# tencent-ailab/pika

Hardware: NVIDIA H100
Metric: utterances/sec RNN-T train step (T=1000,U=150,V=6k) (higher is better)
Workload: dtype bf16

## Files before the change

pika_b200/csrc/common.cuh:

```cuda
#pragma once
#include <cuda.h>
#include <cuda_bf16.h>
#include <cuda_runtime.h>
#include <stdint.h>

#define PK_DEVICE __device__ __forceinline__

namespace pk {

void set_last_error(const char* fmt, ...);
#define PK_CHECK_ARG(cond, msg)                                       \
    do {                                                              \
        if (!(cond)) {                                                \
            pk::set_last_error("%s:%d: %s", __FILE__, __LINE__, msg); \
            return -1;                                                \
        }                                                             \
    } while (0)
#define PK_CHECK_CUDA(expr)                                                                     \
    do {                                                                                        \
        cudaError_t e__ = (expr);                                                               \
        if (e__ != cudaSuccess) {                                                               \
            pk::set_last_error("%s:%d: CUDA error %s", __FILE__, __LINE__, cudaGetErrorString(e__)); \
            return -2;                                                                          \
        }                                                                                       \
// ... 52 lines not shown
    x ^= x >> 15; x *= 0x85EBCA77u; x ^= x >> 13;
    return ((x & 0xFFFFu) >= thresh16 ? 1u : 0u) | ((x >> 16) >= thresh16 ? 2u : 0u);
}
__host__ __device__ inline uint32_t drop_thresh16_of(float p) {
    if (p <= 0.f) return 0u;
    const double t = (double)p * 65536.0 + 0.5;
    const uint32_t r = t >= 65535.0 ? 65535u : (uint32_t)t;
    return r == 0 ? 1u : r;
}
__host__ __device__ inline float drop_scale16_of(uint32_t thresh16) { return thresh16 ? 1.f / (1.f - (float)thresh16 / 65536.f) : 1.f; }

PK_DEVICE float warp_sum(float v) {
#pragma unroll
    for (int o = 16; o > 0; o >>= 1) v += __shfl_xor_sync(0xffffffffu, v, o);
    return v;
}
PK_DEVICE float warp_max(float v) {
#pragma unroll
    for (int o = 16; o > 0; o >>= 1) v = fmaxf(v, __shfl_xor_sync(0xffffffffu, v, o));
    return v;
}

PK_DEVICE uint32_t smem_u32(const void* p) { return (uint32_t)__cvta_generic_to_shared(p); }

PK_DEVICE bool elect_one() {
    uint32_t pred;
    asm volatile(
        "{\n\t.reg .pred p;\n\t.reg .b32 r;\n\t"
        "elect.sync r|p, 0xffffffff;\n\t"
        "selp.u32 %0, 1, 0, p;\n\t}\n"
        : "=r"(pred));
    return pred != 0;
}

PK_DEVICE void mbar_init(uint64_t* bar, uint32_t count) {
    asm volatile("mbarrier.init.shared::cta.b64 [%0], %1;" ::"r"(smem_u32(bar)), "r"(count));
}
PK_DEVICE void mbar_fence_init() { asm volatile("fence.mbarrier_init.release.cluster;" ::: "memory"); }
PK_DEVICE void mbar_arrive_expect_tx(uint64_t* bar, uint32_t bytes) {
    asm volatile("mbarrier.arrive.expect_tx.shared::cta.b64 _, [%0], %1;" ::"r"(smem_u32(bar)), "r"(bytes)
                 : "memory");
}
PK_DEVICE void mbar_arrive(uint64_t* bar) {
    asm volatile("mbarrier.arrive.shared::cta.b64 _, [%0];" ::"r"(smem_u32(bar)) : "memory");
}
PK_DEVICE bool mbar_try_wait(uint64_t* bar, uint32_t parity) {
    uint32_t done;
    asm volatile(
        "{\n\t.reg .pred p;\n\t"
        "mbarrier.try_wait.parity.shared::cta.b64 p, [%1], %2;\n\t"
        "selp.u32 %0, 1, 0, p;\n\t}\n"
        : "=r"(done)
        : "r"(smem_u32(bar)), "r"(parity)
        : "memory");
    return done != 0;
}
PK_DEVICE void mbar_wait(uint64_t* bar, uint32_t parity) {
    while (!mbar_try_wait(bar, parity)) {
    }
}

PK_DEVICE void tma_prefetch_desc(const CUtensorMap* m) {
    asm volatile("prefetch.tensormap [%0];" ::"l"(reinterpret_cast<uint64_t>(m)) : "memory");
}
PK_DEVICE void tma_load_4d(void* smem_dst, const CUtensorMap* m, uint64_t* bar, int c0, int c1, int c2, int c3) {
    asm volatile(
        "cp.async.bulk.tensor.4d.shared::cluster.global.tile.mbarrier::complete_tx::bytes"
        " [%0], [%1, {%3, %4, %5, %6}], [%2];" ::"r"(smem_u32(smem_dst)),
        "l"(reinterpret_cast<uint64_t>(m)), "r"(smem_u32(bar)), "r"(c0), "r"(c1), "r"(c2), "r"(c3)
        : "memory");
}
PK_DEVICE void tma_load_3d(void* smem_dst, const CUtensorMap* m, uint64_t* bar, int c0, int c1, int c2) {
    asm volatile(
        "cp.async.bulk.tensor.3d.shared::cluster.global.tile.mbarrier::complete_tx::bytes"
        " [%0], [%1, {%3, %4, %5}], [%2];" ::"r"(smem_u32(smem_dst)),
        "l"(reinterpret_cast<uint64_t>(m)), "r"(smem_u32(bar)), "r"(c0), "r"(c1), "r"(c2)
        : "memory");
}
PK_DEVICE void bulk_load(void* smem_dst, const void* gsrc, uint32_t bytes, uint64_t* bar) {
    asm volatile("cp.async.bulk.shared::cluster.global.mbarrier::complete_tx::bytes [%0], [%1], %2, [%3];" ::"r"(smem_u32(smem_dst)),
                 "l"(reinterpret_cast<uint64_t>(gsrc)), "r"(bytes), "r"(smem_u32(bar))
                 : "memory");
}
PK_DEVICE void tma_store_4d(const CUtensorMap* m, const void* smem_src, int c0, int c1, int c2, int c3) {
    asm volatile(
        "cp.async.bulk.tensor.4d.global.shared::cta.tile.bulk_group [%0, {%2, %3, %4, %5}], [%1];" ::"l"(
            reinterpret_cast<uint64_t>(m)),
        "r"(smem_u32(smem_src)), "r"(c0), "r"(c1), "r"(c2), "r"(c3)
        : "memory");
}
PK_DEVICE void tma_reduce_add_4d(const CUtensorMap* m, const void* smem_src, int c0, int c1, int c2, int c3) {
    asm volatile(
        "cp.reduce.async.bulk.tensor.4d.global.shared::cta.add.tile.bulk_group [%0, {%2, %3, %4, %5}], [%1];" ::"l"(
            reinterpret_cast<uint64_t>(m)),
        "r"(smem_u32(smem_src)), "r"(c0), "r"(c1), "r"(c2), "r"(c3)
        : "memory");
}
constexpr uint64_t kL2EvictNormal = 0x1000000000000000ull;
constexpr uint64_t kL2EvictFirst = 0x12F0000000000000ull;
constexpr uint64_t kL2EvictLast = 0x14F0000000000000ull;
PK_DEVICE void tma_load_4d_hint(void* smem_dst, const CUtensorMap* m, uint64_t* bar, int c0, int c1, int c2, int c3, uint64_t pol) {
    asm volatile(
        "cp.async.bulk.tensor.4d.shared::cluster.global.tile.mbarrier::complete_tx::bytes.L2::cache_hint"
        " [%0], [%1, {%3, %4, %5, %6}], [%2], %7;" ::"r"(smem_u32(smem_dst)),
        "l"(reinterpret_cast<uint64_t>(m)), "r"(smem_u32(bar)), "r"(c0), "r"(c1), "r"(c2), "r"(c3), "l"(pol)
        : "memory");
}
PK_DEVICE void tma_store_4d_hint(const CUtensorMap* m, const void* smem_src, int c0, int c1, int c2, int c3, uint64_t pol) {
    asm volatile(
        "cp.async.bulk.tensor.4d.global.shared::cta.tile.bulk_group.L2::cache_hint [%0, {%2, %3, %4, %5}], [%1], %6;" ::"l"(
            reinterpret_cast<uint64_t>(m)),
        "r"(smem_u32(smem_src)), "r"(c0), "r"(c1), "r"(c2), "r"(c3), "l"(pol)
        : "memory");
}
PK_DEVICE void tma_store_commit() { asm volatile("cp.async.bulk.commit_group;" ::: "memory"); }
template <int N> PK_DEVICE void tma_store_wait_read() {
    asm volatile("cp.async.bulk.wait_group.read %0;" ::"n"(N) : "memory");
}
template <int N> PK_DEVICE void tma_store_wait() { asm volatile("cp.async.bulk.wait_group %0;" ::"n"(N) : "memory"); }
PK_DEVICE void fence_proxy_async_smem() { asm volatile("fence.proxy.async.shared::cta;" ::: "memory"); }

PK_DEVICE uint64_t make_smem_desc_sw128(uint32_t smem_addr, uint32_t lbo_bytes, uint32_t sbo_bytes) {
    uint64_t d = 0;
    d |= (uint64_t)((smem_addr >> 4) & 0x3FFF);
    d |= (uint64_t)((lbo_bytes >> 4) & 0x3FFF) << 16;
    d |= (uint64_t)((sbo_bytes >> 4) & 0x3FFF) << 32;
    d |= (uint64_t)1 << 62;
    return d;
}
PK_DEVICE void wgmma_fence() { asm volatile("wgmma.fence.sync.aligned;" ::: "memory"); }
PK_DEVICE void wgmma_commit() { asm volatile("wgmma.commit_group.sync.aligned;" ::: "memory"); }
template <int N> PK_DEVICE void wgmma_wait() { asm volatile("wgmma.wait_group.sync.aligned %0;" ::"n"(N) : "memory"); }
template <int R> PK_DEVICE void wgmma_fence_acc(float (&d)[R]) {
#pragma unroll
    for (int i = 0; i < R; ++i) asm volatile("" : "+f"(d[i])::"memory");
}
template <int N> PK_DEVICE void setmaxnreg_inc() { asm volatile("setmaxnreg.inc.sync.aligned.u32 %0;" ::"n"(N)); }
template <int N> PK_DEVICE void setmaxnreg_dec() { asm volatile("setmaxnreg.dec.sync.aligned.u32 %0;" ::"n"(N)); }

template <int TA, int TB> PK_DEVICE void wgmma_ss_n64(float (&d)[32], uint64_t a, uint64_t b, uint32_t acc) {
    asm volatile(
        "{\n\t.reg .pred p;\n\tsetp.ne.b32 p, %34, 0;\n\t"
        "wgmma.mma_async.sync.aligned.m64n64k16.f32.bf16.bf16 {%0, %1, %2, %3, %4, %5, %6, %7, %8, %9, %10, %11, %12, %13, %14, %15, %16, %17, %18, %19, %20, %21, %22, %23, %24, %25, %26, %27, %28, %29, %30, %31}, %32, %33, p, 1, 1, %35, %36;\n\t}\n"
        : "+f"(d[0]), "+f"(d[1]), "+f"(d[2]), "+f"(d[3]), "+f"(d[4]), "+f"(d[5]), "+f"(d[6]), "+f"(d[7]), "+f"(d[8]), "+f"(d[9]), "+f"(d[10]), "+f"(d[11]), "+f"(d[12]), "+f"(d[13]), "+f"(d[14]), "+f"(d[15]), "+f"(d[16]), "+f"(d[17]), "+f"(d[18]), "+f"(d[19]), "+f"(d[20]), "+f"(d[21]), "+f"(d[22]), "+f"(d[23]), "+f"(d[24]), "+f"(d[25]), "+f"(d[26]), "+f"(d[27]), "+f"(d[28]), "+f"(d[29]), "+f"(d[30]), "+f"(d[31])
        : "l"(a), "l"(b), "r"(acc), "n"(TA), "n"(TB));
}
template <int TB> PK_DEVICE void wgmma_rs_n64(float (&d)[32], const uint32_t (&a)[4], uint64_t b, uint32_t acc) {
    asm volatile(
        "{\n\t.reg .pred p;\n\tsetp.ne.b32 p, %37, 0;\n\t"
        "wgmma.mma_async.sync.aligned.m64n64k16.f32.bf16.bf16 {%0, %1, %2, %3, %4, %5, %6, %7, %8, %9, %10, %11, %12, %13, %14, %15, %16, %17, %18, %19, %20, %21, %22, %23, %24, %25, %26, %27, %28, %29, %30, %31}, {%32, %33, %34, %35}, %36, p, 1, 1, %38;\n\t}\n"
        : "+f"(d[0]), "+f"(d[1]), "+f"(d[2]), "+f"(d[3]), "+f"(d[4]), "+f"(d[5]), "+f"(d[6]), "+f"(d[7]), "+f"(d[8]), "+f"(d[9]), "+f"(d[10]), "+f"(d[11]), "+f"(d[12]), "+f"(d[13]), "+f"(d[14]), "+f"(d[15]), "+f"(d[16]), "+f"(d[17]), "+f"(d[18]), "+f"(d[19]), "+f"(d[20]), "+f"(d[21]), "+f"(d[22]), "+f"(d[23]), "+f"(d[24]), "+f"(d[25]), "+f"(d[26]), "+f"(d[27]), "+f"(d[28]), "+f"(d[29]), "+f"(d[30]), "+f"(d[31])
        : "r"(a[0]), "r"(a[1]), "r"(a[2]), "r"(a[3]), "l"(b), "r"(acc), "n"(TB));
}
template <int TA, int TB> PK_DEVICE void wgmma_ss_n128(float (&d)[64], uint64_t a, uint64_t b, uint32_t acc) {
    asm volatile(
        "{\n\t.reg .pred p;\n\tsetp.ne.b32 p, %66, 0;\n\t"
        "wgmma.mma_async.sync.aligned.m64n128k16.f32.bf16.bf16 {%0, %1, %2, %3, %4, %5, %6, %7, %8, %9, %10, %11, %12, %13, %14, %15, %16, %17, %18, %19, %20, %21, %22, %23, %24, %25, %26, %27, %28, %29, %30, %31, %32, %33, %34, %35, %36, %37, %38, %39, %40, %41, %42, %43, %44, %45, %46, %47, %48, %49, %50, %51, %52, %53, %54, %55, %56, %57, %58, %59, %60, %61, %62, %63}, %64, %65, p, 1, 1, %67, %68;\n\t}\n"
        : "+f"(d[0]), "+f"(d[1]), "+f"(d[2]), "+f"(d[3]), "+f"(d[4]), "+f"(d[5]), "+f"(d[6]), "+f"(d[7]), "+f"(d[8]), "+f"(d[9]), "+f"(d[10]), "+f"(d[11]), "+f"(d[12]), "+f"(d[13]), "+f"(d[14]), "+f"(d[15]), "+f"(d[16]), "+f"(d[17]), "+f"(d[18]), "+f"(d[19]), "+f"(d[20]), "+f"(d[21]), "+f"(d[22]), "+f"(d[23]), "+f"(d[24]), "+f"(d[25]), "+f"(d[26]), "+f"(d[27]), "+f"(d[28]), "+f"(d[29]), "+f"(d[30]), "+f"(d[31]), "+f"(d[32]), "+f"(d[33]), "+f"(d[34]), "+f"(d[35]), "+f"(d[36]), "+f"(d[37]), "+f"(d[38]), "+f"(d[39]), "+f"(d[40]), "+f"(d[41]), "+f"(d[42]), "+f"(d[43]), "+f"(d[44]), "+f"(d[45]), "+f"(d[46]), "+f"(d[47]), "+f"(d[48]), "+f"(d[49]), "+f"(d[50]), "+f"(d[51]), "+f"(d[52]), "+f"(d[53]), "+f"(d[54]), "+f"(d[55]), "+f"(d[56]), "+f"(d[57]), "+f"(d[58]), "+f"(d[59]), "+f"(d[60]), "+f"(d[61]), "+f"(d[62]), "+f"(d[63])
        : "l"(a), "l"(b), "r"(acc), "n"(TA), "n"(TB));
}
template <int TA, int TB> PK_DEVICE void wgmma_ss_n256(float (&d)[128], uint64_t a, uint64_t b, uint32_t acc) {
    asm volatile(
        "{\n\t.reg .pred p;\n\tsetp.ne.b32 p, %130, 0;\n\t"
        "wgmma.mma_async.sync.aligned.m64n256k16.f32.bf16.bf16 {%0, %1, %2, %3, %4, %5, %6, %7, %8, %9, %10, %11, %12, %13, %14, %15, %16, %17, %18, %19, %20, %21, %22, %23, %24, %25, %26, %27, %28, %29, %30, %31, %32, %33, %34, %35, %36, %37, %38, %39, %40, %41, %42, %43, %44, %45, %46, %47, %48, %49, %50, %51, %52, %53, %54, %55, %56, %57, %58, %59, %60, %61, %62, %63, %64, %65, %66, %67, %68, %69, %70, %71, %72, %73, %74, %75, %76, %77, %78, %79, %80, %81, %82, %83, %84, %85, %86, %87, %88, %89, %90, %91, %92, %93, %94, %95, %96, %97, %98, %99, %100, %101, %102, %103, %104, %105, %106, %107, %108, %109, %110, %111, %112, %113, %114, %115, %116, %117, %118, %119, %120, %121, %122, %123, %124, %125, %126, %127}, %128, %129, p, 1, 1, %131, %132;\n\t}\n"
        : "+f"(d[0]), "+f"(d[1]), "+f"(d[2]), "+f"(d[3]), "+f"(d[4]), "+f"(d[5]), "+f"(d[6]), "+f"(d[7]), "+f"(d[8]), "+f"(d[9]), "+f"(d[10]), "+f"(d[11]), "+f"(d[12]), "+f"(d[13]), "+f"(d[14]), "+f"(d[15]), "+f"(d[16]), "+f"(d[17]), "+f"(d[18]), "+f"(d[19]), "+f"(d[20]), "+f"(d[21]), "+f"(d[22]), "+f"(d[23]), "+f"(d[24]), "+f"(d[25]), "+f"(d[26]), "+f"(d[27]), "+f"(d[28]), "+f"(d[29]), "+f"(d[30]), "+f"(d[31]), "+f"(d[32]), "+f"(d[33]), "+f"(d[34]), "+f"(d[35]), "+f"(d[36]), "+f"(d[37]), "+f"(d[38]), "+f"(d[39]), "+f"(d[40]), "+f"(d[41]), "+f"(d[42]), "+f"(d[43]), "+f"(d[44]), "+f"(d[45]), "+f"(d[46]), "+f"(d[47]), "+f"(d[48]), "+f"(d[49]), "+f"(d[50]), "+f"(d[51]), "+f"(d[52]), "+f"(d[53]), "+f"(d[54]), "+f"(d[55]), "+f"(d[56]), "+f"(d[57]), "+f"(d[58]), "+f"(d[59]), "+f"(d[60]), "+f"(d[61]), "+f"(d[62]), "+f"(d[63]), "+f"(d[64]), "+f"(d[65]), "+f"(d[66]), "+f"(d[67]), "+f"(d[68]), "+f"(d[69]), "+f"(d[70]), "+f"(d[71]), "+f"(d[72]), "+f"(d[73]), "+f"(d[74]), "+f"(d[75]), "+f"(d[76]), "+f"(d[77]), "+f"(d[78]), "+f"(d[79]), "+f"(d[80]), "+f"(d[81]), "+f"(d[82]), "+f"(d[83]), "+f"(d[84]), "+f"(d[85]), "+f"(d[86]), "+f"(d[87]), "+f"(d[88]), "+f"(d[89]), "+f"(d[90]), "+f"(d[91]), "+f"(d[92]), "+f"(d[93]), "+f"(d[94]), "+f"(d[95]), "+f"(d[96]), "+f"(d[97]), "+f"(d[98]), "+f"(d[99]), "+f"(d[100]), "+f"(d[101]), "+f"(d[102]), "+f"(d[103]), "+f"(d[104]), "+f"(d[105]), "+f"(d[106]), "+f"(d[107]), "+f"(d[108]), "+f"(d[109]), "+f"(d[110]), "+f"(d[111]), "+f"(d[112]), "+f"(d[113]), "+f"(d[114]), "+f"(d[115]), "+f"(d[116]), "+f"(d[117]), "+f"(d[118]), "+f"(d[119]), "+f"(d[120]), "+f"(d[121]), "+f"(d[122]), "+f"(d[123]), "+f"(d[124]), "+f"(d[125]), "+f"(d[126]), "+f"(d[127])
        : "l"(a), "l"(b), "r"(acc), "n"(TA), "n"(TB));
// ... 99 lines not shown
```

pika_b200/csrc/rnnt_loss.cu:

```cuda
#include <algorithm>
#include <cstdlib>

#include "../../include/pika_b200.h"
#include "common.cuh"

namespace pk {
void count_launch();

constexpr float kLog2e = 1.4426950408889634f;
constexpr float kLn2 = 0.6931471805599453f;

template <typename T> struct Vec16;
template <> struct Vec16<__nv_bfloat16> {
    static constexpr int N = 8;
    PK_DEVICE static void unpack(const uint4& q, float (&f)[8]) {
        f[0] = bf16lo(q.x); f[1] = bf16hi(q.x); f[2] = bf16lo(q.y); f[3] = bf16hi(q.y);
        f[4] = bf16lo(q.z); f[5] = bf16hi(q.z); f[6] = bf16lo(q.w); f[7] = bf16hi(q.w);
    }
    PK_DEVICE static uint4 pack(const float (&f)[8]) {
        return make_uint4(pack_bf16x2(f[0], f[1]), pack_bf16x2(f[2], f[3]), pack_bf16x2(f[4], f[5]), pack_bf16x2(f[6], f[7]));
    }
    PK_DEVICE static float vmax(const uint4& q) {
        const __nv_bfloat162 a = __hmax2(*reinterpret_cast<const __nv_bfloat162*>(&q.x), *reinterpret_cast<const __nv_bfloat162*>(&q.y));
        const __nv_bfloat162 b = __hmax2(*reinterpret_cast<const __nv_bfloat162*>(&q.z), *reinterpret_cast<const __nv_bfloat162*>(&q.w));
// ... 295 lines not shown
    for (int o = 1; o < 32; o <<= 1) {
        const int y = __shfl_up_sync(0xffffffffu, x, o);
        if (lane >= o) x += y;
    }
    if (lane == 31) s_warp[w] = x;
    __syncthreads();
    if (w == 0) {
        int s = s_warp[lane];
#pragma unroll
        for (int o = 1; o < 32; o <<= 1) {
            const int y = __shfl_up_sync(0xffffffffu, s, o);
            if (lane >= o) s += y;
        }
        s_warp[lane] = s;
    }
    __syncthreads();
    const int r = x - v + (w > 0 ? s_warp[w - 1] : 0);
    *total = s_warp[31];
    __syncthreads();
    return r;
}

PK_DEVICE int tile_kept(const float* gb, const float* gl, long long rows, long long r0, bool (&keep)[SCAN_PER_THREAD]) {
    int n = 0;
#pragma unroll
    for (int k = 0; k < SCAN_PER_THREAD; ++k) {
        const long long r = r0 + (long long)threadIdx.x * SCAN_PER_THREAD + k;
        keep[k] = r < rows && grad_row_kept(gb[r], gl[r]);
        n += keep[k];
    }
    return n;
}

__global__ void __launch_bounds__(SCAN_THREADS) grad_rows_count_kernel(const float* __restrict__ gb, const float* __restrict__ gl,
                                                                       long long rows, int* __restrict__ tile_count) {
    __shared__ int s_warp[32];
    bool keep[SCAN_PER_THREAD];
    int total;
    block_exclusive_scan(tile_kept(gb, gl, rows, (long long)blockIdx.x * SCAN_TILE, keep), s_warp, &total);
    if (threadIdx.x == 0) tile_count[blockIdx.x] = total;
}

template <typename T>
__global__ void __launch_bounds__(SCAN_THREADS) grad_rows_scan_kernel(int* __restrict__ tile_count, int n_tiles, int* __restrict__ count,
                                                                      long long rows, T* dz_c, int ldv, T* h_c, int H) {
    __shared__ int s_warp[32];
    __shared__ int s_carry;
    if (threadIdx.x == 0) s_carry = 0;
    __syncthreads();
    for (int i0 = 0; i0 < n_tiles; i0 += SCAN_THREADS) {
        const int i = i0 + threadIdx.x;
        const int v = i < n_tiles ? tile_count[i] : 0;
        int total;
        const int ex = block_exclusive_scan(v, s_warp, &total);
        if (i < n_tiles) tile_count[i] = s_carry + ex;
        __syncthreads();
        if (threadIdx.x == 0) s_carry += total;
        __syncthreads();
    }
    const long long kept = s_carry;
    if (threadIdx.x == 0) *count = (int)kept;
    const long long tail = min(rows, (kept + 63) / 64 * 64);
    for (long long r = kept; r < tail; ++r) {
        for (int c = threadIdx.x; c < ldv; c += SCAN_THREADS) dz_c[r * ldv + c] = from_f32<T>(0.f);
        for (int c = threadIdx.x; c < H; c += SCAN_THREADS) h_c[r * H + c] = from_f32<T>(0.f);
    }
}

__global__ void __launch_bounds__(SCAN_THREADS) grad_rows_map_kernel(const float* __restrict__ gb, const float* __restrict__ gl,
                                                                     long long rows, const int* __restrict__ tile_off, int* __restrict__ map) {
    __shared__ int s_warp[32];
    bool keep[SCAN_PER_THREAD];
    const long long r0 = (long long)blockIdx.x * SCAN_TILE;
    int total;
    int idx = tile_off[blockIdx.x] + block_exclusive_scan(tile_kept(gb, gl, rows, r0, keep), s_warp, &total);
#pragma unroll
    for (int k = 0; k < SCAN_PER_THREAD; ++k) {
        const long long r = r0 + (long long)threadIdx.x * SCAN_PER_THREAD + k;
        if (r < rows) map[r] = keep[k] ? idx++ : -1;
    }
}

constexpr int GRAD_THREADS = 256;
template <typename T> struct GradCfg { static constexpr int MAXG = 32 / Vec16<T>::N; };
template <typename T, int GRAD_RU, int MINB, bool COMPACT, bool ROWY = false>
__global__ void __launch_bounds__(GRAD_THREADS, MINB) rnnt_grad_kernel(const T* logits, const int* __restrict__ labels,
                                                                    const int* __restrict__ label_lens, RnntDims d,
                                                                    const float* __restrict__ lse_in, const float* __restrict__ gb_in,
                                                                    const float* __restrict__ gl_in, T* dlogits, float* __restrict__ colsum,
                                                                    long long rows_per_cta, const int* __restrict__ row_map,
                                                                    const T* __restrict__ h, T* __restrict__ h_c, int H,
                                                                    const int* __restrict__ row_y = nullptr) {
    constexpr int VN = Vec16<T>::N;
    constexpr int GRAD_MAXG = GradCfg<T>::MAXG;
    extern __shared__ float gsm[];
    float* s_gb = gsm;
    float* s_gl = gsm + rows_per_cta;
    float* s_l2 = gsm + 2 * rows_per_cta;
    int* s_y = reinterpret_cast<int*>(gsm + 3 * rows_per_cta);
    int* s_map = reinterpret_cast<int*>(gsm + 4 * rows_per_cta);
    const long long rows = (long long)d.B * d.T * d.U1;
    const long long r0 = (long long)blockIdx.x * rows_per_cta;
    const long long r1 = min(rows, r0 + rows_per_cta);
    const int nvec_ld = d.ldv / VN;
    const int tid = threadIdx.x;
    for (long long row = r0 + tid; row < r1; row += GRAD_THREADS) {
        const int i = (int)(row - r0);
        s_gb[i] = gb_in[row];
        s_gl[i] = gl_in[row];
        s_l2[i] = lse_in[row] * kLog2e;
        if (ROWY) {
            s_y[i] = row_y[row];
        } else {
            const int u = (int)(row % d.U1);
            const int b = (int)(row / ((long long)d.T * d.U1));
            s_y[i] = (u < label_lens[b]) ? labels[(size_t)b * d.ld_labels + u] : -1;
        }
        if (COMPACT) s_map[i] = row_map[row];
    }
    __syncthreads();
    const int h_vec = COMPACT ? H / 8 : 0;
    float cs[GRAD_MAXG][VN];
#pragma unroll
    for (int gq = 0; gq < GRAD_MAXG; ++gq)
#pragma unroll
        for (int e = 0; e < VN; ++e) cs[gq][e] = 0.f;
    for (long long rb = r0; rb < r1; rb += GRAD_RU) {
        uint4 q[GRAD_RU][GRAD_MAXG];
        uint4 hq[GRAD_RU];
#pragma unroll
        for (int k = 0; k < GRAD_RU; ++k) {
            const long long row = rb + k;
            if (row < r1 && (COMPACT ? s_map[row - r0] >= 0 : (s_gb[row - r0] != 0.f || s_gl[row - r0] != 0.f))) {
                const uint4* vp = reinterpret_cast<const uint4*>(logits + row * (long long)d.ldv);
#pragma unroll
                for (int gq = 0; gq < GRAD_MAXG; ++gq) {
                    const int i = tid + gq * GRAD_THREADS;
                    if (i < nvec_ld) q[k][gq] = ld_plain(vp + i);
                }
                if (COMPACT && tid < h_vec) hq[k] = ld_stream(reinterpret_cast<const uint4*>(h + row * (long long)H) + tid);
            }
        }
#pragma unroll
        for (int k = 0; k < GRAD_RU; ++k) {
            const long long row = rb + k;
            if (row >= r1) continue;
            const float gb = s_gb[row - r0], gl = s_gl[row - r0];
            long long orow = row;
            if (COMPACT) {
                orow = s_map[row - r0];
                if (orow < 0) continue;
                if (tid < h_vec) st_stream(reinterpret_cast<uint4*>(h_c + orow * H) + tid, hq[k]);
            }
            uint4* op = reinterpret_cast<uint4*>(dlogits + orow * (long long)d.ldv);
            if (gb == 0.f && gl == 0.f) {
#pragma unroll
                for (int gq = 0; gq < GRAD_MAXG; ++gq) {
                    const int i = tid + gq * GRAD_THREADS;
                    if (i < nvec_ld) st_stream(op + i, make_uint4(0, 0, 0, 0));
                }
                continue;
            }
            const int y = s_y[row - r0];
            const float l2 = s_l2[row - r0];
            const float gsum = -(gb + gl);
#pragma unroll
            for (int gq = 0; gq < GRAD_MAXG; ++gq) {
                const int i = tid + gq * GRAD_THREADS;
                if (i < nvec_ld) {
                    float f[VN];
                    Vec16<T>::unpack(q[k][gq], f);
#pragma unroll
                    for (int e = 0; e < VN; ++e) f[e] = ex2_approx(fmaf(f[e], kLog2e, -l2)) * gsum;
                    const int v0 = i * VN;
                    if (v0 == 0) f[0] += gb;
                    if (y >= v0 && y < v0 + VN) {
#pragma unroll
                        for (int e = 0; e < VN; ++e) if (v0 + e == y) f[e] += gl;
                    }
                    if (v0 + VN > d.V) {
#pragma unroll
                        for (int e = 0; e < VN; ++e) if (v0 + e >= d.V) f[e] = 0.f;
                    }
                    const uint4 packed = Vec16<T>::pack(f);
                    st_stream(op + i, packed);
                    if (colsum) {
                        float w[VN];
                        Vec16<T>::unpack(packed, w);
#pragma unroll
                        for (int e = 0; e < VN; ++e) cs[gq][e] += w[e];
                    }
                }
            }
        }
    }
    if (colsum) {
        float* part = colsum + (size_t)blockIdx.x * d.ldv;
#pragma unroll
        for (int gq = 0; gq < GRAD_MAXG; ++gq) {
            const int i = tid + gq * GRAD_THREADS;
            if (i < nvec_ld) {
#pragma unroll
                for (int e = 0; e < VN; ++e) part[i * VN + e] = cs[gq][e];
            }
        }
    }
}

__global__ void __launch_bounds__(256) colsum_partials_kernel(const float* __restrict__ part, int n_part, int ld, float* __restrict__ out) {
    __shared__ float sm[8][33];
    const int tx = threadIdx.x & 31, ty = threadIdx.x >> 5;
    const int c = blockIdx.x * 32 + tx;
    float a = 0.f;
    if (c < ld) {
        const int per = (n_part + 7) / 8;
        const int i0 = ty * per, i1 = min(n_part, i0 + per);
        float a0 = 0.f, a1 = 0.f, a2 = 0.f, a3 = 0.f;
        int i = i0;
        for (; i + 4 <= i1; i += 4) {
            a0 += part[(size_t)(i + 0) * ld + c]; a1 += part[(size_t)(i + 1) * ld + c];
            a2 += part[(size_t)(i + 2) * ld + c]; a3 += part[(size_t)(i + 3) * ld + c];
        }
        for (; i < i1; ++i) a0 += part[(size_t)i * ld + c];
        a = (a0 + a1) + (a2 + a3);
    }
    sm[ty][tx] = a;
    __syncthreads();
    if (ty == 0 && c < ld) {
        float t = sm[0][tx];
#pragma unroll
        for (int k = 1; k < 8; ++k) t += sm[k][tx];
        out[c] = t;
    }
}

template <typename T>
__global__ void __launch_bounds__(256) pruned_row_lse_kernel(const T* __restrict__ logits, const int* __restrict__ frame_lens,
                                                             const int* __restrict__ label_lens, const int* __restrict__ bounds, int Tt,
                                                             int R, int V, int ldv, long long rows, const float2* __restrict__ parts,
                                                             int n_parts, float* __restrict__ lse_out) {
    constexpr int VN = Vec16<T>::N;
    const int lane = threadIdx.x & 31;
    const long long n_warps = (long long)gridDim.x * (blockDim.x >> 5);
    for (long long row = (long long)blockIdx.x * (blockDim.x >> 5) + (threadIdx.x >> 5); row < rows; row += n_warps) {
        const long long bt = row / R;
        const int r = (int)(row - bt * R), t = (int)(bt % Tt), b = (int)(bt / Tt);
        if (t >= frame_lens[b] || bounds[bt] < 0 || bounds[bt] + r > label_lens[b]) continue;
        float lse;
        if (parts != nullptr) {
            float m = -INFINITY, sum = 0.f;
            for (int i = 0; i < n_parts; ++i) m = fmaxf(m, parts[(size_t)i * rows + row].x);
            for (int i = 0; i < n_parts; ++i) { const float2 ps = parts[(size_t)i * rows + row]; sum += ps.y * exp2f(ps.x - m); }
            lse = (m + log2f(sum)) * kLn2;
        } else {
            const T* rp = logits + row * (long long)ldv;
            float m = -INFINITY, sum = 0.f;
            const int nfull = V / VN;
            for (int i = lane; i < nfull; i += 32) {
                float f[VN];
                Vec16<T>::unpack(ld_plain(reinterpret_cast<const uint4*>(rp) + i), f);
#pragma unroll
                for (int e = 0; e < VN; ++e) {
                    const float x = f[e] * kLog2e;
                    if (x > m) { sum *= exp2f(m - x); m = x; }
                    sum += exp2f(x - m);
                }
            }
            for (int v = nfull * VN + lane; v < V; v += 32) {
                const float x = to_f32<T>(rp[v]) * kLog2e;
                if (x > m) { sum *= exp2f(m - x); m = x; }
                sum += exp2f(x - m);
            }
            const float mw = warp_max(m);
            sum = (m == -INFINITY) ? 0.f : sum * exp2f(m - mw);
            sum = warp_sum(sum);
            lse = (mw + log2f(sum)) * kLn2;
        }
        if (lane == 0) lse_out[row] = lse;
    }
}

template <typename T>
__global__ void __launch_bounds__(256) pruned_tables_kernel(const T* __restrict__ logits, const int* __restrict__ labels,
                                                            const int* __restrict__ frame_lens, const int* __restrict__ label_lens,
                                                            const int* __restrict__ bounds, RnntDims d, int R,
                                                            const float* __restrict__ lse, float* __restrict__ lpb_skew,
                                                            float* __restrict__ lpl_skew) {
    const long long n = (long long)d.B * d.T * d.U1;
    for (long long i = (long long)blockIdx.x * blockDim.x + threadIdx.x; i < n; i += (long long)gridDim.x * blockDim.x) {
// ... 71 lines not shown
    PK_CHECK_ARG(cpt <= LAT_MAX_CPT, "U too large for the lattice kernel (U+1 <= 2048)");
    static bool configured = false;
    if (!configured) {
        PK_CHECK_CUDA(cudaFuncSetAttribute(rnnt_lattice_kernel, cudaFuncAttributeMaxDynamicSharedMemorySize,
                                           2 * 2 * (LAT_MAX_G * LAT_MAX_CPT + 2) * (int)sizeof(lat_t)));
        configured = true;
    }
    rnnt_lattice_kernel<<<d.B, 2 * G, lat_smem, stream>>>(frame_lens, label_lens, d, G, cpt, lpb, lpl, alpha, beta, grad_scale,
                                                       costs, gb, gl);
    PK_CHECK_LAUNCH(); count_launch();
    return 0;
}

static int rnnt_loss_impl(const void* logits, int dtype, const int* labels, const int* frame_lens,
                          const int* label_lens, int B, int T, int U1, int V, int ldv, int ld_labels,
                          const float* grad_scale, float* costs, void* dlogits, float* dlogits_colsum, void* workspace,
                          long long workspace_bytes, const float* row_lse, int n_parts, int* row_map, int* row_count,
                          const void* h, int H, void* h_c, void* stream_v) {
    using namespace pk;
    cudaStream_t stream = reinterpret_cast<cudaStream_t>(stream_v);
    PK_CHECK_ARG(dtype == PK_F32 || dtype == PK_BF16, "bad dtype");
    PK_CHECK_ARG(B > 0 && T > 0 && U1 > 0 && V > 1, "bad dims");
    const int vn = dtype == PK_F32 ? 4 : 8;
    PK_CHECK_ARG(ldv >= V && ldv % vn == 0, "ldv must be >= V and a multiple of 16 bytes");
    PK_CHECK_ARG((reinterpret_cast<uintptr_t>(logits) & 15) == 0, "logits not 16B aligned");
    PK_CHECK_ARG(dlogits == nullptr || (reinterpret_cast<uintptr_t>(dlogits) & 15) == 0, "dlogits not 16B aligned");
    PK_CHECK_ARG(workspace_bytes >= pk_rnnt_loss_workspace_bytes(B, T, U1), "workspace too small");
    RnntDims d{B, T, U1, V, ldv, ld_labels, T + U1 - 1};
    const size_t skew = (size_t)B * d.ND * U1, nodes = (size_t)B * T * U1;
    double* wsd = reinterpret_cast<double*>(workspace);
    double* alpha = wsd; double* beta = alpha + skew;
    float* lpb = reinterpret_cast<float*>(beta + skew); float* lpl = lpb + skew;
    float* lse = lpl + skew; float* gb = lse + nodes; float* gl = gb + nodes;

    const long long rows = (long long)nodes;
    const int warps_per_cta = 8;
    long long want = (rows + warps_per_cta - 1) / warps_per_cta;
    const long long cap = (long long)num_sms() * 8 * 4;
    const int grid = (int)(want < cap ? want : cap);
    if (row_lse != nullptr) {
        PK_CHECK_ARG(n_parts >= 1, "n_parts must be >= 1");
        const int fgrid = (int)((rows + 255) / 256 < (long long)num_sms() * 8 ? (rows + 255) / 256 : (long long)num_sms() * 8);
        if (dtype == PK_BF16)
            rnnt_rowfinish_kernel<__nv_bfloat16><<<fgrid, 256, 0, stream>>>(reinterpret_cast<const __nv_bfloat16*>(logits), labels, frame_lens,
                                                                           label_lens, d, reinterpret_cast<const float2*>(row_lse), n_parts,
                                                                           lse, lpb, lpl);
        else
            rnnt_rowfinish_kernel<float><<<fgrid, 256, 0, stream>>>(reinterpret_cast<const float*>(logits), labels, frame_lens, label_lens, d,
                                                                   reinterpret_cast<const float2*>(row_lse), n_parts, lse, lpb, lpl);
    } else if (dtype == PK_BF16)
        rnnt_rowstats_kernel<__nv_bfloat16><<<grid, 256, 0, stream>>>(reinterpret_cast<const __nv_bfloat16*>(logits), labels,
                                                                     frame_lens, label_lens, d, lse, lpb, lpl);
    else
        rnnt_rowstats_kernel<float><<<grid, 256, 0, stream>>>(reinterpret_cast<const float*>(logits), labels, frame_lens,
                                                              label_lens, d, lse, lpb, lpl);
    PK_CHECK_LAUNCH(); count_launch();
    {
        const int rc = launch_lattice(frame_lens, label_lens, d, lpb, lpl, alpha, beta, grad_scale, costs, gb, gl, stream);
        if (rc) return rc;
    }
    if (dlogits != nullptr) {
        PK_CHECK_ARG(ldv <= 8192, "V too large for the gradient kernel (V <= 8192)");
        int ggrid; long long rpc;
        rnnt_grad_grid(rows, &rpc, &ggrid);
        float* cs_part = nullptr;
        if (dlogits_colsum) {
            const long long base_bytes = pk_rnnt_loss_workspace_bytes(B, T, U1);
            PK_CHECK_ARG(workspace_bytes >= base_bytes + (long long)ggrid * ldv * 4,
                         "workspace too small for the column sums (add pk_rnnt_loss_colsum_workspace_bytes)");
            cs_part = reinterpret_cast<float*>(reinterpret_cast<unsigned char*>(workspace) + base_bytes);
        }
        if (row_map != nullptr) {
            const int n_tiles = (int)((rows + SCAN_TILE - 1) / SCAN_TILE);
            int* tile_count = reinterpret_cast<int*>(alpha);
            grad_rows_count_kernel<<<n_tiles, SCAN_THREADS, 0, stream>>>(gb, gl, rows, tile_count);
            PK_CHECK_LAUNCH(); count_launch();
            grad_rows_scan_kernel<__nv_bfloat16><<<1, SCAN_THREADS, 0, stream>>>(tile_count, n_tiles, row_count, rows,
                                                                                 reinterpret_cast<__nv_bfloat16*>(dlogits), ldv,
                                                                                 reinterpret_cast<__nv_bfloat16*>(h_c), H);
            PK_CHECK_LAUNCH(); count_launch();
            grad_rows_map_kernel<<<n_tiles, SCAN_THREADS, 0, stream>>>(gb, gl, rows, tile_count, row_map);
            PK_CHECK_LAUNCH(); count_launch();
        }
        const size_t gsmem = (size_t)rpc * (row_map != nullptr ? 20 : 16);
#define PK_GRAD_LAUNCH(TT, RU, MB, CP)                                                                                     \
        rnnt_grad_kernel<TT, RU, MB, CP><<<ggrid, GRAD_THREADS, gsmem, stream>>>(reinterpret_cast<const TT*>(logits), labels, label_lens, d, \
                                                                                lse, gb, gl, reinterpret_cast<TT*>(dlogits), cs_part, rpc,  \
                                                                                row_map, reinterpret_cast<const TT*>(h),                    \
                                                                                reinterpret_cast<TT*>(h_c), H)
        if (row_map != nullptr) PK_GRAD_LAUNCH(__nv_bfloat16, 2, 3, true);
        else if (dtype == PK_BF16) PK_GRAD_LAUNCH(__nv_bfloat16, 2, 3, false);
        else PK_GRAD_LAUNCH(float, 2, 2, false);
#undef PK_GRAD_LAUNCH
        PK_CHECK_LAUNCH(); count_launch();
        if (dlogits_colsum) {
            colsum_partials_kernel<<<(ldv + 31) / 32, 256, 0, stream>>>(cs_part, ggrid, ldv, dlogits_colsum);
            PK_CHECK_LAUNCH(); count_launch();
        }
    }
    return 0;
}

extern "C" int pk_rnnt_loss_fwd_bwd(const void* logits, int dtype, const int* labels, const int* frame_lens,
                                    const int* label_lens, int B, int T, int U1, int V, int ldv, int ld_labels,
                                    const float* grad_scale, float* costs, void* dlogits, float* dlogits_colsum, void* workspace,
                                    long long workspace_bytes, void* stream) {
    return rnnt_loss_impl(logits, dtype, labels, frame_lens, label_lens, B, T, U1, V, ldv, ld_labels, grad_scale, costs, dlogits,
                          dlogits_colsum, workspace, workspace_bytes, nullptr, 0, nullptr, nullptr, nullptr, 0, nullptr, stream);
}

extern "C" int pk_rnnt_loss_fwd_bwd_lse(const void* logits, int dtype, const int* labels, const int* frame_lens,
                                        const int* label_lens, int B, int T, int U1, int V, int ldv, int ld_labels,
                                        const float* grad_scale, float* costs, void* dlogits, float* dlogits_colsum, void* workspace,
                                        long long workspace_bytes, const float* row_lse, int n_parts, void* stream) {
    PK_CHECK_ARG(row_lse != nullptr, "row_lse is null");
    return rnnt_loss_impl(logits, dtype, labels, frame_lens, label_lens, B, T, U1, V, ldv, ld_labels, grad_scale, costs, dlogits,
                          dlogits_colsum, workspace, workspace_bytes, row_lse, n_parts, nullptr, nullptr, nullptr, 0, nullptr, stream);
}

extern "C" int pk_rnnt_loss_fwd_bwd_compact(const void* logits, int dtype, const int* labels, const int* frame_lens,
                                            const int* label_lens, int B, int T, int U1, int V, int ldv, int ld_labels,
                                            const float* grad_scale, float* costs, void* dz_c, float* dlogits_colsum, void* workspace,
                                            long long workspace_bytes, const float* row_lse, int n_parts, const void* h, int H,
                                            void* h_c, int* row_map, int* row_count, void* stream) {
    PK_CHECK_ARG(dtype == PK_BF16, "the compacted gradient is bf16 only");
    PK_CHECK_ARG(dz_c != nullptr && row_map != nullptr && row_count != nullptr && h != nullptr && h_c != nullptr, "null pointer");
    PK_CHECK_ARG(H > 0 && H % 8 == 0 && H / 8 <= pk::GRAD_THREADS, "H must be a multiple of 8, <= 2048");
    PK_CHECK_ARG(dz_c != logits, "dz_c must not alias the logits");
    PK_CHECK_ARG((reinterpret_cast<uintptr_t>(h) & 15) == 0 && (reinterpret_cast<uintptr_t>(h_c) & 15) == 0, "h / h_c not 16B aligned");
    return rnnt_loss_impl(logits, dtype, labels, frame_lens, label_lens, B, T, U1, V, ldv, ld_labels, grad_scale, costs, dz_c,
                          dlogits_colsum, workspace, workspace_bytes, row_lse, n_parts, row_map, row_count, h, H, h_c, stream);
}

static long long lattice_ws_bytes(int B, int T, int U1) { return 2 * (long long)B * ((long long)T + U1 - 1) * U1 * 8; }
extern "C" int pk_rnnt_lattice_workspace(int B, int T, int U1, long long* bytes) {
    PK_CHECK_ARG(B > 0 && T > 0 && U1 > 0 && bytes != nullptr, "bad dims or null pointer");
    *bytes = lattice_ws_bytes(B, T, U1);
    return 0;
}

extern "C" int pk_rnnt_lattice(const int* frame_lens, const int* label_lens, int B, int T, int U1, const float* lpb_skew,
                               const float* lpl_skew, const float* grad_scale, float* costs, float* gb, float* gl, void* workspace,
                               long long workspace_bytes, void* stream) {
    using namespace pk;
    PK_CHECK_ARG(B > 0 && T > 0 && U1 > 0, "bad dims");
    PK_CHECK_ARG(lpb_skew && lpl_skew && costs && gb && gl && workspace, "null pointer");
    PK_CHECK_ARG(workspace_bytes >= lattice_ws_bytes(B, T, U1), "workspace too small");
    RnntDims d{B, T, U1, 2, 2, 1, T + U1 - 1};
    const size_t skew = (size_t)B * d.ND * U1;
    double* alpha = reinterpret_cast<double*>(workspace);
    return launch_lattice(frame_lens, label_lens, d, lpb_skew, lpl_skew, alpha, alpha + skew, grad_scale, costs, gb, gl,
                          reinterpret_cast<cudaStream_t>(stream));
}

static long long pruned_ws_parts(int B, int T, int U1, int R, int ldv, long long* colsum_off) {
    const long long skew = (long long)B * ((long long)T + U1 - 1) * U1, nodes = (long long)B * T * U1, rows = (long long)B * T * R;
    const long long base = 2 * skew * 8 + 2 * skew * 4 + 2 * nodes * 4 + 4 * rows * 4;
    const long long off = (base + 255) / 256 * 256;
    int ggrid; long long rpc;
    rnnt_grad_grid(rows, &rpc, &ggrid);
    if (colsum_off) *colsum_off = off;
    return off + (long long)ggrid * ldv * 4;
}
extern "C" int pk_rnnt_pruned_loss_workspace(int B, int T, int U1, int R, int ldv, long long* bytes) {
    PK_CHECK_ARG(B > 0 && T > 0 && U1 > 0 && R >= 1 && ldv > 0 && bytes != nullptr, "bad dims or null pointer");
    *bytes = pruned_ws_parts(B, T, U1, R, ldv, nullptr);
    return 0;
}

extern "C" int pk_rnnt_pruned_loss(const void* logits, int dtype, const int* labels, const int* frame_lens, const int* label_lens,
                                   const int* bounds, int B, int T, int U1, int R, int V, int ldv, int ld_labels, const float* grad_scale,
                                   float* costs, void* dlogits, float* dlogits_colsum, void* workspace, long long workspace_bytes,
                                   const float* row_lse, int n_parts, void* stream_v) {
    using namespace pk;
    cudaStream_t stream = reinterpret_cast<cudaStream_t>(stream_v);
    PK_CHECK_ARG(dtype == PK_F32 || dtype == PK_BF16, "bad dtype");
    PK_CHECK_ARG(B > 0 && T > 0 && U1 > 0 && R >= 1 && V > 1, "bad dims");
    const int vn = dtype == PK_F32 ? 4 : 8;
    PK_CHECK_ARG(ldv >= V && ldv % vn == 0, "ldv must be >= V and a multiple of 16 bytes");
    PK_CHECK_ARG((reinterpret_cast<uintptr_t>(logits) & 15) == 0, "logits not 16B aligned");
    PK_CHECK_ARG(dlogits == nullptr || (reinterpret_cast<uintptr_t>(dlogits) & 15) == 0, "dlogits not 16B aligned");
    PK_CHECK_ARG(row_lse == nullptr || n_parts >= 1, "n_parts must be >= 1");
    long long cs_off;
    PK_CHECK_ARG(workspace_bytes >= pruned_ws_parts(B, T, U1, R, ldv, &cs_off), "workspace too small");
    RnntDims d{B, T, U1, V, ldv, ld_labels, T + U1 - 1};
    const size_t skew = (size_t)B * d.ND * U1, nodes = (size_t)B * T * U1;
    const long long rows = (long long)B * T * R;
    double* alpha = reinterpret_cast<double*>(workspace); double* beta = alpha + skew;
    float* lpb = reinterpret_cast<float*>(beta + skew); float* lpl = lpb + skew;
    float* gb = lpl + skew; float* gl = gb + nodes;
    float* lse = gl + nodes; float* gb_row = lse + rows; float* gl_row = gb_row + rows;
    int* y_row = reinterpret_cast<int*>(gl_row + rows);
    const int wgrid = (int)std::min<long long>((rows + 7) / 8, (long long)num_sms() * 32);
    const long long nn = (long long)B * T * U1;
    const int ngrid = (int)std::min<long long>((nn + 255) / 256, (long long)num_sms() * 8);
    if (dtype == PK_BF16) {
        using TT = __nv_bfloat16;
        pruned_row_lse_kernel<TT><<<wgrid, 256, 0, stream>>>((const TT*)logits, frame_lens, label_lens, bounds, T, R, V, ldv, rows,
                                                            (const float2*)row_lse, n_parts, lse);
        PK_CHECK_LAUNCH(); count_launch();
        pruned_tables_kernel<TT><<<ngrid, 256, 0, stream>>>((const TT*)logits, labels, frame_lens, label_lens, bounds, d, R, lse, lpb, lpl);
    } else {
        pruned_row_lse_kernel<float><<<wgrid, 256, 0, stream>>>((const float*)logits, frame_lens, label_lens, bounds, T, R, V, ldv, rows,
                                                               (const float2*)row_lse, n_parts, lse);
        PK_CHECK_LAUNCH(); count_launch();
        pruned_tables_kernel<float><<<ngrid, 256, 0, stream>>>((const float*)logits, labels, frame_lens, label_lens, bounds, d, R, lse, lpb, lpl);
    }
    PK_CHECK_LAUNCH(); count_launch();
    {
        const int rc = launch_lattice(frame_lens, label_lens, d, lpb, lpl, alpha, beta, grad_scale, costs, gb, gl, stream);
        if (rc) return rc;
    }
    if (dlogits == nullptr) return 0;
    PK_CHECK_ARG(ldv <= 8192, "V too large for the gradient kernel (V <= 8192)");
    const int rgrid = (int)std::min<long long>((rows + 255) / 256, (long long)num_sms() * 8);
    pruned_rows_kernel<<<rgrid, 256, 0, stream>>>(labels, frame_lens, label_lens, bounds, d, R, gb, gl, gb_row, gl_row, y_row);
    PK_CHECK_LAUNCH(); count_launch();
    int ggrid; long long rpc;
    rnnt_grad_grid(rows, &rpc, &ggrid);
    float* cs_part = dlogits_colsum ? reinterpret_cast<float*>(reinterpret_cast<unsigned char*>(workspace) + cs_off) : nullptr;
    RnntDims dr{B, T, R, V, ldv, ld_labels, 0};
    const size_t gsmem = (size_t)rpc * 16;
    if (dtype == PK_BF16)
        rnnt_grad_kernel<__nv_bfloat16, 2, 3, false, true><<<ggrid, GRAD_THREADS, gsmem, stream>>>(
            (const __nv_bfloat16*)logits, labels, label_lens, dr, lse, gb_row, gl_row, (__nv_bfloat16*)dlogits, cs_part, rpc, nullptr,
            nullptr, nullptr, 0, y_row);
    else
        rnnt_grad_kernel<float, 2, 2, false, true><<<ggrid, GRAD_THREADS, gsmem, stream>>>(
            (const float*)logits, labels, label_lens, dr, lse, gb_row, gl_row, (float*)dlogits, cs_part, rpc, nullptr, nullptr, nullptr, 0,
            y_row);
    PK_CHECK_LAUNCH(); count_launch();
    if (dlogits_colsum) {
        colsum_partials_kernel<<<(ldv + 31) / 32, 256, 0, stream>>>(cs_part, ggrid, ldv, dlogits_colsum);
        PK_CHECK_LAUNCH(); count_launch();
    }
    return 0;
}
```

Before: 288.3.

## Stream RNN-T gradient rows through a TMA bulk-copy smem ring buffer

Replaces the register-unrolled per-thread global loads and streaming stores in the RNN-T gradient kernel with a multi-slot shared-memory ring. One thread issues bulk async loads of each active logits row (and h row when compacting) ahead of use, waiting on mbarriers. Results are written back in place to smem and sent out with bulk async stores. The aim is deeper memory-level parallelism and overlap of load, compute and store in a bandwidth-bound kernel. In exchange it adds a CTA-wide barrier per row, a single-thread issue path and larger dynamic shared memory, which may reduce occupancy.

```diff
diff --git a/pika_b200/csrc/common.cuh b/pika_b200/csrc/common.cuh
--- a/pika_b200/csrc/common.cuh
+++ b/pika_b200/csrc/common.cuh
@@ -158,6 +158,11 @@
                  "l"(reinterpret_cast<uint64_t>(gsrc)), "r"(bytes), "r"(smem_u32(bar))
                  : "memory");
 }
+PK_DEVICE void bulk_store(void* gdst, const void* smem_src, uint32_t bytes) {
+    asm volatile("cp.async.bulk.global.shared::cta.bulk_group [%0], [%1], %2;" ::"l"(reinterpret_cast<uint64_t>(gdst)),
+                 "r"(smem_u32(smem_src)), "r"(bytes)
+                 : "memory");
+}
 PK_DEVICE void tma_store_4d(const CUtensorMap* m, const void* smem_src, int c0, int c1, int c2, int c3) {
     asm volatile(
         "cp.async.bulk.tensor.4d.global.shared::cta.tile.bulk_group [%0, {%2, %3, %4, %5}], [%1];" ::"l"(
diff --git a/pika_b200/csrc/rnnt_loss.cu b/pika_b200/csrc/rnnt_loss.cu
--- a/pika_b200/csrc/rnnt_loss.cu
+++ b/pika_b200/csrc/rnnt_loss.cu
@@ -401,28 +401,40 @@
 }
 
 constexpr int GRAD_THREADS = 256;
+constexpr int GRAD_MAX_SLOTS = 8;
 template <typename T> struct GradCfg { static constexpr int MAXG = 32 / Vec16<T>::N; };
-template <typename T, int GRAD_RU, int MINB, bool COMPACT, bool ROWY = false>
+__host__ __device__ inline long long grad_scalar_bytes(long long rpc, bool compact) { return (rpc * (compact ? 20 : 16) + 127) / 128 * 128; }
+inline long long grad_slot_bytes(int ldv, int elem_bytes, int H) { return ((long long)ldv * elem_bytes + 2LL * H + 127) / 128 * 128; }
+template <typename T, int MINB, bool COMPACT, bool ROWY = false>
 __global__ void __launch_bounds__(GRAD_THREADS, MINB) rnnt_grad_kernel(const T* logits, const int* __restrict__ labels,
                                                                     const int* __restrict__ label_lens, RnntDims d,
                                                                     const float* __restrict__ lse_in, const float* __restrict__ gb_in,
                                                                     const float* __restrict__ gl_in, T* dlogits, float* __restrict__ colsum,
-                                                                    long long rows_per_cta, const int* __restrict__ row_map,
+                                                                    long long rows_per_cta, int n_slots, const int* __restrict__ row_map,
                                                                     const T* __restrict__ h, T* __restrict__ h_c, int H,
                                                                     const int* __restrict__ row_y = nullptr) {
     constexpr int VN = Vec16<T>::N;
     constexpr int GRAD_MAXG = GradCfg<T>::MAXG;
-    extern __shared__ float gsm[];
+    extern __shared__ __align__(128) float gsm[];
+    __shared__ uint64_t full[GRAD_MAX_SLOTS];
     float* s_gb = gsm;
     float* s_gl = gsm + rows_per_cta;
     float* s_l2 = gsm + 2 * rows_per_cta;
     int* s_y = reinterpret_cast<int*>(gsm + 3 * rows_per_cta);
     int* s_map = reinterpret_cast<int*>(gsm + 4 * rows_per_cta);
+    const uint32_t row_bytes = (uint32_t)d.ldv * sizeof(T);
+    const uint32_t h_bytes = COMPACT ? (uint32_t)H * sizeof(T) : 0u;
+    uint8_t* ring = reinterpret_cast<uint8_t*>(gsm) + grad_scalar_bytes(rows_per_cta, COMPACT);
+    const uint32_t slot_bytes = (row_bytes + h_bytes + 127) / 128 * 128;
     const long long rows = (long long)d.B * d.T * d.U1;
     const long long r0 = (long long)blockIdx.x * rows_per_cta;
     const long long r1 = min(rows, r0 + rows_per_cta);
     const int nvec_ld = d.ldv / VN;
     const int tid = threadIdx.x;
+    if (tid == 0) {
+        for (int s = 0; s < n_slots; ++s) mbar_init(&full[s], 1);
+        mbar_fence_init();
+    }
     for (long long row = r0 + tid; row < r1; row += GRAD_THREADS) {
         const int i = (int)(row - r0);
         s_gb[i] = gb_in[row];
@@ -438,92 +450,119 @@
         if (COMPACT) s_map[i] = row_map[row];
     }
     __syncthreads();
-    const int h_vec = COMPACT ? H / 8 : 0;
+    auto streamed = [&](int i) { return COMPACT ? s_map[i] >= 0 : (s_gb[i] != 0.f || s_gl[i] != 0.f); };
+    long long ld_row = r0;
+    auto fill = [&](int slot) {
+        while (ld_row < r1 && !streamed((int)(ld_row - r0))) ++ld_row;
+        if (ld_row >= r1) return;
+        uint8_t* sp = ring + (size_t)slot * slot_bytes;
+        mbar_arrive_expect_tx(&full[slot], row_bytes + h_bytes);
+        bulk_load(sp, logits + ld_row * (long long)d.ldv, row_bytes, &full[slot]);
+        if (COMPACT) bulk_load(sp + row_bytes, h + ld_row * (long long)H, h_bytes, &full[slot]);
+        ++ld_row;
+    };
+    if (tid == 0)
+        for (int s = 0; s + 1 < n_slots; ++s) fill(s);
     float cs[GRAD_MAXG][VN];
 #pragma unroll
     for (int gq = 0; gq < GRAD_MAXG; ++gq)
 #pragma unroll
         for (int e = 0; e < VN; ++e) cs[gq][e] = 0.f;
-    for (long long rb = r0; rb < r1; rb += GRAD_RU) {
-        uint4 q[GRAD_RU][GRAD_MAXG];
-        uint4 hq[GRAD_RU];
-#pragma unroll
-        for (int k = 0; k < GRAD_RU; ++k) {
-            const long long row = rb + k;
-            if (row < r1 && (COMPACT ? s_map[row - r0] >= 0 : (s_gb[row - r0] != 0.f || s_gl[row - r0] != 0.f))) {
-                const uint4* vp = reinterpret_cast<const uint4*>(logits + row * (long long)d.ldv);
-#pragma unroll
-                for (int gq = 0; gq < GRAD_MAXG; ++gq) {
-                    const int i = tid + gq * GRAD_THREADS;
-                    if (i < nvec_ld) q[k][gq] = ld_plain(vp + i);
-                }
-                if (COMPACT && tid < h_vec) hq[k] = ld_stream(reinterpret_cast<const uint4*>(h + row * (long long)H) + tid);
-            }
-        }
-#pragma unroll
-        for (int k = 0; k < GRAD_RU; ++k) {
-            const long long row = rb + k;
-            if (row >= r1) continue;
-            const float gb = s_gb[row - r0], gl = s_gl[row - r0];
-            long long orow = row;
-            if (COMPACT) {
-                orow = s_map[row - r0];
-                if (orow < 0) continue;
-                if (tid < h_vec) st_stream(reinterpret_cast<uint4*>(h_c + orow * H) + tid, hq[k]);
-            }
-            uint4* op = reinterpret_cast<uint4*>(dlogits + orow * (long long)d.ldv);
-            if (gb == 0.f && gl == 0.f) {
+    int n = 0;
+    for (long long row = r0; row < r1; ++row) {
+        const int ri = (int)(row - r0);
+        const float gb = s_gb[ri], gl = s_gl[ri];
+        if (!streamed(ri)) {
+            if (!COMPACT) {
+                uint4* op = reinterpret_cast<uint4*>(dlogits + row * (long long)d.ldv);
 #pragma unroll
                 for (int gq = 0; gq < GRAD_MAXG; ++gq) {
                     const int i = tid + gq * GRAD_THREADS;
                     if (i < nvec_ld) st_stream(op + i, make_uint4(0, 0, 0, 0));
                 }
-                continue;
-            }
-            const int y = s_y[row - r0];
-            const float l2 = s_l2[row - r0];
-            const float gsum = -(gb + gl);
-#pragma unroll
-            for (int gq = 0; gq < GRAD_MAXG; ++gq) {
-                const int i = tid + gq * GRAD_THREADS;
-                if (i < nvec_ld) {
-                    float f[VN];
-                    Vec16<T>::unpack(q[k][gq], f);
-#pragma unroll
-                    for (int e = 0; e < VN; ++e) f[e] = ex2_approx(fmaf(f[e], kLog2e, -l2)) * gsum;
-                    const int v0 = i * VN;
-                    if (v0 == 0) f[0] += gb;
-                    if (y >= v0 && y < v0 + VN) {
-#pragma unroll
-                        for (int e = 0; e < VN; ++e) if (v0 + e == y) f[e] += gl;
-                    }
-                    if (v0 + VN > d.V) {
-#pragma unroll
-                        for (int e = 0; e < VN; ++e) if (v0 + e >= d.V) f[e] = 0.f;
-                    }
-                    const uint4 packed = Vec16<T>::pack(f);
-                    st_stream(op + i, packed);
-                    if (colsum) {
-                        float w[VN];
-                        Vec16<T>::unpack(packed, w);
-#pragma unroll
-                        for (int e = 0; e < VN; ++e) cs[gq][e] += w[e];
-                    }
-                }
-            }
-        }
-    }
-    if (colsum) {
-        float* part = colsum + (size_t)blockIdx.x * d.ldv;
+            }
+            continue;
+        }
+        const int slot = n % n_slots;
+        uint8_t* sp = ring + (size_t)slot * slot_bytes;
+        const uint32_t sa = smem_u32(sp);
+        mbar_wait(&full[slot], (uint32_t)(n / n_slots) & 1u);
+        const int y = s_y[ri];
+        const float l2 = s_l2[ri];
+        const float gsum = -(gb + gl);
 #pragma unroll
         for (int gq = 0; gq < GRAD_MAXG; ++gq) {
             const int i = tid + gq * GRAD_THREADS;
             if (i < nvec_ld) {
+                float f[VN];
+                Vec16<T>::unpack(lds_u32x4(sa + 16u * i), f);
+#pragma unroll
+                for (int e = 0; e < VN; ++e) f[e] = ex2_approx(fmaf(f[e], kLog2e, -l2)) * gsum;
+                const int v0 = i * VN;
+                if (v0 == 0) f[0] += gb;
+                if (y >= v0 && y < v0 + VN) {
+#pragma unroll
+                    for (int e = 0; e < VN; ++e) if (v0 + e == y) f[e] += gl;
+                }
+                if (v0 + VN > d.V) {
+#pragma unroll
+                    for (int e = 0; e < VN; ++e) if (v0 + e >= d.V) f[e] = 0.f;
+                }
+                const uint4 packed = Vec16<T>::pack(f);
+                *reinterpret_cast<uint4*>(sp + 16 * i) = packed;
+                if (colsum) {
+                    float w[VN];
+                    Vec16<T>::unpack(packed, w);
+#pragma unroll
+                    for (int e = 0; e < VN; ++e) cs[gq][e] += w[e];
+                }
+            }
+        }
+        fence_proxy_async_smem();
+        __syncthreads();
+        if (tid == 0) {
+            const long long orow = COMPACT ? (long long)s_map[ri] : row;
+            bulk_store(dlogits + orow * (long long)d.ldv, sp, row_bytes);
+            if (COMPACT) bulk_store(h_c + orow * (long long)H, sp + row_bytes, h_bytes);
+            tma_store_commit();
+            tma_store_wait_read<1>();
+            fill((n + n_slots - 1) % n_slots);
+        }
+        ++n;
+    }
+    if (tid == 0) tma_store_wait_read<0>();
+    if (colsum) {
+        float* part = colsum + (size_t)blockIdx.x * d.ldv;
+#pragma unroll
+        for (int gq = 0; gq < GRAD_MAXG; ++gq) {
+            const int i = tid + gq * GRAD_THREADS;
+            if (i < nvec_ld) {
 #pragma unroll
                 for (int e = 0; e < VN; ++e) part[i * VN + e] = cs[gq][e];
             }
         }
     }
+}
+
+template <typename T, int MINB, bool COMPACT, bool ROWY = false>
+static int launch_grad(int ggrid, cudaStream_t stream, const T* logits, const int* labels, const int* label_lens, const RnntDims& d,
+                        const float* lse, const float* gb, const float* gl, T* dlogits, float* colsum, long long rpc,
+                        const int* row_map, const T* h, T* h_c, int H, const int* row_y) {
+    constexpr long long kSmemPerSm = 228 * 1024, kReservedPerCta = 1024, kStatic = 128;
+    const long long scalars = grad_scalar_bytes(rpc, COMPACT);
+    const long long slot = grad_slot_bytes(d.ldv, (int)sizeof(T), COMPACT ? H : 0);
+    const long long budget = kSmemPerSm / MINB - kReservedPerCta - kStatic - scalars;
+    const int n_slots = (int)std::max(2LL, std::min((long long)GRAD_MAX_SLOTS, budget / slot));
+    const long long smem = scalars + n_slots * slot;
+    static long long configured = 48 * 1024;
+    if (smem > configured) {
+        PK_CHECK_CUDA(cudaFuncSetAttribute(rnnt_grad_kernel<T, MINB, COMPACT, ROWY>, cudaFuncAttributeMaxDynamicSharedMemorySize, (int)smem));
+        configured = smem;
+    }
+    rnnt_grad_kernel<T, MINB, COMPACT, ROWY><<<ggrid, GRAD_THREADS, smem, stream>>>(
+        logits, labels, label_lens, d, lse, gb, gl, dlogits, colsum, rpc, n_slots, row_map, h, h_c, H, row_y);
+    PK_CHECK_LAUNCH();
+    return 0;
 }
 
 __global__ void __launch_bounds__(256) colsum_partials_kernel(const float* __restrict__ part, int n_part, int ld, float* __restrict__ out) {
@@ -761,17 +800,19 @@
             grad_rows_map_kernel<<<n_tiles, SCAN_THREADS, 0, stream>>>(gb, gl, rows, tile_count, row_map);
             PK_CHECK_LAUNCH(); count_launch();
         }
-        const size_t gsmem = (size_t)rpc * (row_map != nullptr ? 20 : 16);
-#define PK_GRAD_LAUNCH(TT, RU, MB, CP)                                                                                     \
-        rnnt_grad_kernel<TT, RU, MB, CP><<<ggrid, GRAD_THREADS, gsmem, stream>>>(reinterpret_cast<const TT*>(logits), labels, label_lens, d, \
-                                                                                lse, gb, gl, reinterpret_cast<TT*>(dlogits), cs_part, rpc,  \
-                                                                                row_map, reinterpret_cast<const TT*>(h),                    \
-                                                                                reinterpret_cast<TT*>(h_c), H)
-        if (row_map != nullptr) PK_GRAD_LAUNCH(__nv_bfloat16, 2, 3, true);
-        else if (dtype == PK_BF16) PK_GRAD_LAUNCH(__nv_bfloat16, 2, 3, false);
-        else PK_GRAD_LAUNCH(float, 2, 2, false);
-#undef PK_GRAD_LAUNCH
-        PK_CHECK_LAUNCH(); count_launch();
+        using BF = __nv_bfloat16;
+        int rc;
+        if (row_map != nullptr)
+            rc = launch_grad<BF, 3, true>(ggrid, stream, (const BF*)logits, labels, label_lens, d, lse, gb, gl, (BF*)dlogits, cs_part, rpc,
+                                          row_map, (const BF*)h, (BF*)h_c, H, nullptr);
+        else if (dtype == PK_BF16)
+            rc = launch_grad<BF, 3, false>(ggrid, stream, (const BF*)logits, labels, label_lens, d, lse, gb, gl, (BF*)dlogits, cs_part, rpc,
+                                           nullptr, nullptr, nullptr, 0, nullptr);
+        else
+            rc = launch_grad<float, 2, false>(ggrid, stream, (const float*)logits, labels, label_lens, d, lse, gb, gl, (float*)dlogits,
+                                              cs_part, rpc, nullptr, nullptr, nullptr, 0, nullptr);
+        if (rc) return rc;
+        count_launch();
         if (dlogits_colsum) {
             colsum_partials_kernel<<<(ldv + 31) / 32, 256, 0, stream>>>(cs_part, ggrid, ldv, dlogits_colsum);
             PK_CHECK_LAUNCH(); count_launch();
@@ -899,16 +940,14 @@
     rnnt_grad_grid(rows, &rpc, &ggrid);
     float* cs_part = dlogits_colsum ? reinterpret_cast<float*>(reinterpret_cast<unsigned char*>(workspace) + cs_off) : nullptr;
     RnntDims dr{B, T, R, V, ldv, ld_labels, 0};
-    const size_t gsmem = (size_t)rpc * 16;
-    if (dtype == PK_BF16)
-        rnnt_grad_kernel<__nv_bfloat16, 2, 3, false, true><<<ggrid, GRAD_THREADS, gsmem, stream>>>(
-            (const __nv_bfloat16*)logits, labels, label_lens, dr, lse, gb_row, gl_row, (__nv_bfloat16*)dlogits, cs_part, rpc, nullptr,
-            nullptr, nullptr, 0, y_row);
-    else
-        rnnt_grad_kernel<float, 2, 2, false, true><<<ggrid, GRAD_THREADS, gsmem, stream>>>(
-            (const float*)logits, labels, label_lens, dr, lse, gb_row, gl_row, (float*)dlogits, cs_part, rpc, nullptr, nullptr, nullptr, 0,
-            y_row);
-    PK_CHECK_LAUNCH(); count_launch();
+    const int rc = dtype == PK_BF16
+                       ? launch_grad<__nv_bfloat16, 3, false, true>(ggrid, stream, (const __nv_bfloat16*)logits, labels, label_lens, dr, lse,
+                                                                    gb_row, gl_row, (__nv_bfloat16*)dlogits, cs_part, rpc, nullptr, nullptr,
+                                                                    nullptr, 0, y_row)
+                       : launch_grad<float, 2, false, true>(ggrid, stream, (const float*)logits, labels, label_lens, dr, lse, gb_row, gl_row,
+                                                            (float*)dlogits, cs_part, rpc, nullptr, nullptr, nullptr, 0, y_row);
+    if (rc) return rc;
+    count_launch();
     if (dlogits_colsum) {
         colsum_partials_kernel<<<(ldv + 31) / 32, 256, 0, stream>>>(cs_part, ggrid, ldv, dlogits_colsum);
         PK_CHECK_LAUNCH(); count_launch();
```

After: 291.1, median of 6. About the same (+1.0%).
